# grayhong/self-diagnosing-gan

Hardware: AMD Instinct MI355X
Metric: images/sec (G+D step) (higher is better)
Workload: dtype f32

## Files before the change

self-diagnosing-gan_amd/csrc/train_ops.hip:

```cpp
#include "common.h"

namespace diagan {

enum LossType : int { LOSS_GAN = 0, LOSS_NS = 1, LOSS_HINGE = 2, LOSS_WASSERSTEIN = 3 };

__device__ __forceinline__ float softplus_f(float x) { return fmaxf(x, 0.f) + log1pf(expf(-fabsf(x))); }
__device__ __forceinline__ float sigmoid_f(float x) { return 1.f / (1.f + expf(-x)); }

__device__ __forceinline__ double block_sum_d(double v, double* red) {
  v = wave_sum(v);
  __syncthreads();
  if ((threadIdx.x & 63) == 0) red[threadIdx.x >> 6] = v;
  __syncthreads();
  return (red[0] + red[1]) + (red[2] + red[3]);
}

__global__ __launch_bounds__(256) void d_loss_kernel(const float* __restrict__ real, int n_real,
                                                     const float* __restrict__ fake, int n_fake, int loss_type,
                                                     int gold, float* __restrict__ d_real, float* __restrict__ d_fake,
                                                     float* __restrict__ out) {
  __shared__ double red[4];
  double lr = 0, lf = 0, pr = 0, pf = 0;
  for (int i = threadIdx.x; i < n_real; i += 256) {
    const float x = real[i], s = sigmoid_f(x);
    float l, g;
    if (loss_type == LOSS_HINGE) { l = fmaxf(1.f - x, 0.f); g = x < 1.f ? -1.f : 0.f; }
    else if (loss_type == LOSS_WASSERSTEIN) { l = -x; g = -1.f; }
    else { l = softplus_f(-x); g = s - 1.f; }
    lr += l; pr += s;
    if (d_real) d_real[i] = g / (float)n_real;
  }
  for (int i = threadIdx.x; i < n_fake; i += 256) {
    const float x = fake[i], s = sigmoid_f(x);
    float l, g;
    if (loss_type == LOSS_HINGE) { l = fmaxf(1.f + x, 0.f); g = x > -1.f ? 1.f : 0.f; }
    else if (loss_type == LOSS_WASSERSTEIN) { l = x; g = 1.f; }
    else { l = softplus_f(x); g = s; }
    if (gold) { l *= x; g *= x; }
    lf += l; pf += s;
    if (d_fake) d_fake[i] = g / (float)n_fake;
  }
  lr = block_sum_d(lr, red); lf = block_sum_d(lf, red);
  pr = block_sum_d(pr, red); pf = block_sum_d(pf, red);
  if (threadIdx.x == 0) {
    out[0] = (float)(lr / n_real) + (float)(lf / n_fake);
    out[1] = (float)(pr / n_real);
    out[2] = (float)(pf / n_fake);
  }
}

__global__ __launch_bounds__(256) void g_loss_kernel(const float* __restrict__ fake, int n, int k, int loss_type,
                                                     float* __restrict__ d_fake, float* __restrict__ out) {
  __shared__ double red[4];
  double ls = 0;
  for (int i = threadIdx.x; i < n; i += 256) {
    const float x = fake[i];
    bool sel = true;
    if (k < n) {
      int rank = 0;
      for (int j = 0; j < n; ++j) {
        const float y = fake[j];
        rank += (y > x) || (y == x && j < i);
      }
      sel = rank < k;
    }
    float l = 0.f, g = 0.f;
    if (sel) {
      if (loss_type == LOSS_NS) {
        const float s = sigmoid_f(x);
        l = -logf(s + 1e-8f);
        g = -s * (1.f - s) / (s + 1e-8f);
      } else if (loss_type == LOSS_GAN) {
        l = softplus_f(-x);
        g = sigmoid_f(x) - 1.f;
      }
      else { l = -x; g = -1.f; }
    }
    ls += l;
    if (d_fake) d_fake[i] = g / (float)k;
  }
  ls = block_sum_d(ls, red);
  if (threadIdx.x == 0) out[0] = (float)(ls / k);
}

struct AdamHyper { float lr, beta1, beta2, eps, bc1, bc2_sqrt, grad_scale, pad; };

__global__ __launch_bounds__(256) void adam_kernel(float* __restrict__ p, const float* __restrict__ g,
                                                   float* __restrict__ m, float* __restrict__ v, long n4,
                                                   const AdamHyper h) {
  typedef float f32x4 __attribute__((ext_vector_type(4)));
  const float step_size = h.lr / h.bc1;
  for (long i = (long)blockIdx.x * blockDim.x + threadIdx.x; i < n4; i += (long)gridDim.x * blockDim.x) {
    const f32x4 gv = reinterpret_cast<const f32x4*>(g)[i] * h.grad_scale;
    f32x4 mv = reinterpret_cast<f32x4*>(m)[i], vv = reinterpret_cast<f32x4*>(v)[i], pv = reinterpret_cast<f32x4*>(p)[i];
#pragma unroll
    for (int e = 0; e < 4; ++e) {
      mv[e] = mv[e] + (gv[e] - mv[e]) * (1.f - h.beta1);
      vv[e] = vv[e] * h.beta2 + (1.f - h.beta2) * gv[e] * gv[e];
// ... 78 lines not shown
```

self-diagnosing-gan_amd/diagan/models/base.py:

```python
import os

import torch

from diagan.models.layers import FlatNet
from diagan.ops import eltwise as E


PREFETCH_FAKES = os.environ.get("DIAGAN_PREFETCH_FAKES", "1") != "0"
STACK_G_STEP = os.environ.get("DIAGAN_STACK_G_STEP", "1") != "0"


def _world_size():
    from diagan.trainer import distributed as dist
    return dist.get_world_size()


class BaseModel(FlatNet):

    def restore_checkpoint(self, ckpt_file, optimizer=None):
        if not ckpt_file:
            raise ValueError("No checkpoint file to be restored.")
        ckpt_dict = torch.load(ckpt_file, map_location='cpu', weights_only=False)
        self.load_state_dict(ckpt_dict['model_state_dict'])
        self.param_version += 1
        if optimizer:
            optimizer.load_state_dict(ckpt_dict['optimizer_state_dict'])
        return ckpt_dict['global_step']

    def save_checkpoint(self, directory, global_step, optimizer=None, name=None):
        if not os.path.exists(directory):
            os.makedirs(directory)
        ckpt_dict = {
            'model_state_dict': self.state_dict(),
            'optimizer_state_dict': optimizer.state_dict() if optimizer is not None else None,
            'global_step': global_step,
        }
        if name is None:
            name = "{}_{}_steps.pth".format(os.path.basename(directory), global_step)
        torch.save(ckpt_dict, os.path.join(directory, name))

    def count_params(self):
        return FlatNet.count_params(self)


class BaseGenerator(BaseModel):
    def __init__(self, nz, ngf, bottom_width, loss_type, **kwargs):
        super().__init__()
        self.nz, self.ngf, self.bottom_width, self.loss_type = nz, ngf, bottom_width, loss_type

    def forward(self, x):
        img, _ = self.forward_nhwc(x, self.training, save=False)
        return E.nhwc_to_nchw(img, self.out_channels)

    def generate_images(self, num_images, device=None, noise=None):
        if device is None:
            device = self.device
        if noise is None:
            noise = torch.randn((num_images, self.nz), device=device)
        return self.forward(noise)

    def generate_images_nhwc(self, num_images, device=None, noise=None, save=False, out=None):
        if device is None:
            device = self.device
        if noise is None and not save:
            ready = self._take_prefetched(num_images)
            if ready is not None:
                if out is not None:
                    out.copy_(ready)
                    ready = out
                return ready, None
        if noise is None and save and out is None:
            ready = getattr(self, '_g_step_ready', None)
            self._g_step_ready = None
            if ready is not None and ready[0].shape[0] == num_images and ready[2] == self.param_version and self.training:
                return ready[0], ready[1]
        if noise is None:
            noise = torch.randn((num_images, self.nz), device=device)
        return self.forward_nhwc(noise, self.training, save=save, out=out)

    supports_stacked_forward = False
    max_stacked_images = 0

    def prefetch_fakes(self, count, batch_size, device=None, g_step=False):
        self._fake_pool, self._g_step_ready = [], None
        if not (self.supports_stacked_forward and self.training and count > 1 and PREFETCH_FAKES):
            return
        device = self.device if device is None else device
        per_chunk = min(count, self.max_stacked_images // max(batch_size, 1))
        if per_chunk < 2:
            return
        if g_step and STACK_G_STEP and (count + 1) * batch_size <= self.max_stacked_images:
            noise = [torch.randn((batch_size, self.nz), device=device) for _ in range(count + 1)]
            imgs, ctx = self.forward_nhwc(torch.cat(noise), True, save=True, groups=count + 1, save_group=count)
            parts = imgs.split(batch_size)
            self._fake_pool.extend(parts[:count])
            self._fake_pool_version = self.param_version
            self._g_step_ready = (parts[count], ctx, self.param_version)
            return
        noise = [torch.randn((batch_size, self.nz), device=device) for _ in range(count)]
        for lo in range(0, count, per_chunk):
            part = noise[lo: lo + per_chunk]
            imgs, _ = self.forward_nhwc(torch.cat(part), True, save=False, groups=len(part))
            self._fake_pool.extend(imgs.split(batch_size))
        self._fake_pool_version = self.param_version

    def _take_prefetched(self, num_images):
        pool = getattr(self, '_fake_pool', None)
        if not pool:
            return None
        if pool[0].shape[0] != num_images or self._fake_pool_version != self.param_version or not self.training:
            self._fake_pool = []
            return None
        return pool.pop(0)

    def compute_gan_loss(self, output):
        k = None
        if getattr(self, 'use_topk', False):
            k = int(self.topk_rate * output.shape[0])
        errG, _ = E.loss_gen(output.detach().contiguous(), self.loss_type, k=k, need_grad=False)
        return errG[0]

    def adversarial_grads(self, real_batch, netD, optG, device=None, noise=None):
        self.zero_grad()
        self.wgrad_batch.hold = _world_size() > 1
        batch_size = real_batch[0].shape[0]
        fake, gctx = self.generate_images_nhwc(batch_size, device=device, noise=noise, save=True)
        output, dctx = netD.forward_nhwc(fake, netD.training, save=True, need_dgrad=True, need_in_dgrad=True)
        k = None
        if getattr(self, 'use_topk', False):
            k = int(self.topk_rate * batch_size)
        errG, dlogit = E.loss_gen(output, self.loss_type, k=k)
        g_img = netD.backward_nhwc(dctx, dlogit, need_wgrad=False, need_gx=True)
        self.backward_nhwc(gctx, g_img)
        self.sync_grads(optG)
        return errG

    def train_step(self, real_batch, netD, optG, log_data, device=None, global_step=None, scaler=None, noise=None,
                   **kwargs):
        if scaler is not None:
            raise NotImplementedError("amp/GradScaler is not part of the fp32 MI355X path")
        errG = self.adversarial_grads(real_batch, netD, optG, device=device, noise=noise)
        optG.step()
        log_data.add_metric('errG', errG[0], group='loss')
        return log_data


class BaseDiscriminator(BaseModel):
    supports_defer_step = True

    def __init__(self, ndf, loss_type, **kwargs):
        super().__init__()
        self.ndf, self.loss_type = ndf, loss_type
        self.use_gold = False

    def to_nhwc(self, x):
        return E.nchw_to_nhwc(x.to(dtype=torch.float32), self.in_channels_padded)

    def forward(self, x):
        logit, _ = self.forward_nhwc(self.to_nhwc(x), self.training, save=False, need_dgrad=False)
        return logit

    def compute_gan_loss(self, output_real, output_fake):
        out3, _, _ = E.loss_dis(output_real.detach().contiguous(), output_fake.detach().contiguous(),
                                self.loss_type, gold=self.use_gold, need_grad=False)
        return out3[0]

    def compute_probs(self, output_real, output_fake):
        out3, _, _ = E.loss_dis(output_real.detach().contiguous(), output_fake.detach().contiguous(),
                                self.loss_type, gold=False, need_grad=False)
        return out3[1].item(), out3[2].item()

    def train_step(self, real_batch, netG, optD, log_data, device=None, global_step=None, scaler=None, noise=None,
                   **kwargs):
        if scaler is not None:
            raise NotImplementedError("amp/GradScaler is not part of the fp32 MI355X path")
        self.zero_grad()
        self.wgrad_batch.hold = _world_size() > 1
        real_images = real_batch[0]
        batch_size = real_images.shape[0]
        if getattr(self, 'pair_forward', False) and self.training:
            B, _, H, W = real_images.shape
            x_all = torch.empty((2 * B, H, W, self.in_channels_padded), dtype=torch.float32, device=real_images.device)
            E.nchw_to_nhwc(real_images.to(dtype=torch.float32), self.in_channels_padded, out=x_all[:B])
            netG.generate_images_nhwc(batch_size, device=device, noise=noise, save=False, out=x_all[B:])
            out_all, ctx = self.forward_nhwc(x_all, True, save=True, need_dgrad=True, need_in_dgrad=False, slot='pair')
            dl = torch.empty(2 * B, dtype=torch.float32, device=x_all.device)
            out3, _, _ = E.loss_dis(out_all[:B], out_all[B:], self.loss_type, gold=self.use_gold, d_real=dl[:B],
                                    d_fake=dl[B:])
            self.backward_nhwc(ctx, dl, need_wgrad=True, need_gx=False)
        else:
            out_real, ctx_r = self.forward_nhwc(self.to_nhwc(real_images), self.training, save=True, need_dgrad=True,
                                                need_in_dgrad=False)
            fake, _ = netG.generate_images_nhwc(batch_size, device=device, noise=noise, save=False)
            out_fake, ctx_f = self.forward_nhwc(fake, self.training, save=True, need_dgrad=True, need_in_dgrad=False,
                                                slot=1)
            out3, d_real, d_fake = E.loss_dis(out_real, out_fake, self.loss_type, gold=self.use_gold)
            self.backward_nhwc(ctx_r, d_real, need_wgrad=True, need_gx=False)
            self.backward_nhwc(ctx_f, d_fake, need_wgrad=True, need_gx=False)
        defer = bool(kwargs.get('defer_step', False))
        self.sync_grads(optD, async_op=defer)
        if not defer:
            optD.step()
        log_data.add_metric('errD', out3[0], group='loss')
        log_data.add_metric('D(x)', out3[1], group='prob')
        log_data.add_metric('D(G(z))', out3[2], group='prob')
        return log_data
```

self-diagnosing-gan_amd/diagan/models/layers.py:

```python

import os

import torch
import torch.nn as nn

from diagan.ops import conv as C
from diagan.ops import eltwise as E

WGRAD_BOX = os.environ.get("DIAGAN_WGRAD_BOX", "1") != "0"


def _r4(n):
    return (n + 3) // 4 * 4


class ConvLayer(nn.Module):

    def __init__(self, kind, in_ch, out_ch, ksize, stride=1, pad=0, bias=True, sn=False, xavier_gain=None):
        super().__init__()
        self.kind, self.in_ch, self.out_ch, self.ksize = kind, in_ch, out_ch, ksize
        self.Cip, self.Cop = _r4(in_ch), _r4(out_ch)
        self.geom = C.Geom(kind, self.Cip, self.Cop, ksize, ksize, stride, pad)
        self.sn = sn
        ref = (nn.Conv2d if kind == 'conv' else nn.ConvTranspose2d)(in_ch, out_ch, ksize, stride, pad, bias=bias)
# ... 278 lines not shown
        return self

    def _perm(self, w):
        return w.view(self.ch, self.bw * self.bw, -1).permute(1, 0, 2).reshape(self.ch * self.bw * self.bw, -1)

    def _unperm(self, w):
        return w.view(self.bw * self.bw, self.ch, -1).permute(1, 0, 2).reshape(self.ch * self.bw * self.bw, -1)

    def _pack(self, w):
        out = torch.zeros((w.shape[0], self.geom.Kp), dtype=w.dtype, device=w.device)
        out[:, : self.nz] = self._perm(w)
        return out

    @staticmethod
    def _sd_hook(module, sd, prefix, local_metadata):
        sd[prefix + 'weight'] = module._unperm(sd[prefix + 'weight'][:, : module.nz]).contiguous()
        sd[prefix + 'bias'] = module._unperm(sd[prefix + 'bias'].view(-1, 1)).view(-1).contiguous()
        return sd

    def _load_hook(self, sd, prefix, *args):
        k = prefix + 'weight'
        if k in sd:
            sd[k] = self._pack(sd[k].to(torch.float32))
        if prefix + 'bias' in sd:
            sd[prefix + 'bias'] = self._perm(sd[prefix + 'bias'].to(torch.float32).view(-1, 1)).view(-1).contiguous()
        net = getattr(self, '_net', None)
        if net is not None:
            net.param_version += 1

    def fwd(self, z):
        B = z.shape[0]
        if self.nzp != self.nz:
            z = torch.nn.functional.pad(z, (0, self.nzp - self.nz))
        x = z.contiguous().view(B, 1, 1, self.nzp)
        y = C.conv_fwd(self.geom, x, self.weight.data, bias=self.bias.data)
        return x, y.view(B, self.bw, self.bw, self.ch)

    sn = False

    def wgrad(self, x, dy, slot=0):
        B = x.shape[0]
        dy2 = dy.reshape(B, 1, 1, -1)
        net = getattr(self, '_net', None)
        if net is not None:
            net.wgrad_batch.launch(self, slot, dy2, x, None, None)
            return
        C.conv_wgrad(self.geom, dy2, x, self.weight.grad, accumulate=True)
        E.colsum(dy2, self.bias.grad, accumulate=True)


class HeadLinear(nn.Module):

    def __init__(self, in_ch, sn=True, xavier_gain=None):
        super().__init__()
        self.in_ch, self.sn = in_ch, sn
        ref = nn.Linear(in_ch, 1)
        if xavier_gain is not None:
            nn.init.xavier_uniform_(ref.weight.data, xavier_gain)
        self.weight = nn.Parameter(ref.weight.data.clone())
        self.bias = nn.Parameter(torch.cat([ref.bias.data, torch.zeros(3)]))
        if sn:
            self.register_buffer('sn_u', torch.randn(1, 1))
            self.register_buffer('sn_sigma', torch.ones(1))
        self._register_state_dict_hook(self._sd_hook)
        self._register_load_state_dict_pre_hook(self._load_hook)

    def xavier_(self, gain):
        w = torch.empty(1, self.in_ch)
        nn.init.xavier_uniform_(w, gain)
        self.weight.data.copy_(w.to(self.weight.device))
        return self

    @staticmethod
    def _sd_hook(module, sd, prefix, local_metadata):
        sd[prefix + 'bias'] = sd[prefix + 'bias'][:1].clone()
        return sd

    def _load_hook(self, sd, prefix, *args):
        k = prefix + 'bias'
        if k in sd and sd[k].numel() == 1:
            sd[k] = torch.cat([sd[k].to(torch.float32), torch.zeros(3, device=sd[k].device)])

    class Ctx:
        __slots__ = ("u", "v", "state", "x", "pooled", "_keep", "pair")

        def __init__(self):
            self.pair = None

    def fwd(self, x, training, slot=None):
        ctx = HeadLinear.Ctx()
        inv = None
        if self.sn and slot == 'pair':
            p0, p1 = self._slot_ctx[0], self._slot_ctx[1]
            ctx.pair = (p0, p1)
            ctx.x = x
            ctx.pooled, logit = E.head_fwd(x, self.weight.data, p0.state[1:], self.bias.data, inv_sigma1=p1.state[1:])
            return ctx, logit
        if self.sn and slot is not None:
            pre = self._slot_ctx[slot]
            ctx.u, ctx.v, ctx.state = pre.u, pre.v, pre.state
            inv = ctx.state[1:]
        elif self.sn:
            ctx.u, ctx.v, ctx.state = C.sn_power_iter(self.weight.data, self.sn_u.view(-1), self.sn_sigma,
                                                      training=training)
            inv = ctx.state[1:]
        ctx.x = x
        ctx.pooled, logit = E.head_fwd(x, self.weight.data, inv, self.bias.data)
        return ctx, logit

    def bwd(self, ctx, dlogit, need_wgrad=True):
        if ctx.pair is not None:
            from diagan import _native as nat
            p0, p1 = ctx.pair
            gx, _, _ = E.head_bwd(dlogit, self.weight.data, p0.state[1:], ctx.x, ctx.pooled, need_gx=True,
                                  need_wgrad=False, inv_sigma1=p1.state[1:])
            if need_wgrad:
                h = dlogit.numel() // 2
                for p, sl in ((p0, slice(0, h)), (p1, slice(h, 2 * h))):
                    _, G, dot = E.head_bwd(dlogit[sl], self.weight.data, None, ctx.x[sl], ctx.pooled[sl], need_gx=False,
                                           need_wgrad=True, dbias=self.bias.grad)
                    nat.call("diagan_sn_grad_fix", nat.ptr(G), nat.ptr(dot), 1, nat.ptr(p.u), nat.ptr(p.v),
                             nat.ptr(p.state), nat.ptr(self.weight.grad), 1, self.in_ch, 1, nat.current_stream())
            return gx
        inv = ctx.state[1:] if self.sn else None
        gx, G, dot = E.head_bwd(dlogit, self.weight.data, inv, ctx.x, ctx.pooled, need_gx=True,
                                need_wgrad=need_wgrad, dbias=self.bias.grad if need_wgrad else None)
        if need_wgrad:
            if self.sn:
                from diagan import _native as nat
                nat.call("diagan_sn_grad_fix", nat.ptr(G), nat.ptr(dot), 1, nat.ptr(ctx.u), nat.ptr(ctx.v),
                         nat.ptr(ctx.state), nat.ptr(self.weight.grad), 1, self.in_ch, 1, nat.current_stream())
            else:
                E.add(self.weight.grad.view(-1), G, out=self.weight.grad.view(-1))
        return gx


class SNBatch:

    def __init__(self, net, layers, n_slots=2):
        import numpy as np
        from diagan import _native as nat
        self.net, self.layers, self.nat = net, layers, nat
        dev = net.flat_params.device
        self.slab_generation = net.slab_generation
        desc = np.dtype([('p', np.uint64, 9), ('i', np.int32, 6)])
        self.tables = []
        f32 = dict(dtype=torch.float32, device=dev)
        dims = []
        for slot in range(n_slots):
            tab = np.zeros(len(layers), dtype=desc)
            for li, m in enumerate(layers):
                if isinstance(m, ConvLayer):
                    g = m.geom
                    Co, Ci, RS, Kp, Kd = g.Co, g.Ci, g.R * g.S, g.Kp, g.Kd
                    wf, wd = torch.zeros((Co, Kp), **f32), torch.zeros((Ci, Kd), **f32)
                    ctx = ConvLayer.Ctx()
                else:
                    Co, Ci, RS, Kp, Kd = 1, m.in_ch, 1, m.in_ch, 0
                    wf = wd = None
                    ctx = HeadLinear.Ctx()
                ctx.u, ctx.v, ctx.state = torch.zeros(Co, **f32), torch.zeros(Kp, **f32), torch.ones(2, **f32)
                if isinstance(m, ConvLayer):
                    ctx.wf, ctx.wd, ctx.wkey = wf, wd, slot
                work = torch.zeros(8 * Kp + Co, **f32)
                ctx._keep = (work,)
                if not hasattr(m, '_slot_ctx') or m._slot_ctx is None or len(m._slot_ctx) != n_slots:
                    m._slot_ctx = [None] * n_slots
                m._slot_ctx[slot] = ctx
                ptrs = [m.weight.data.data_ptr(), m.sn_u.data_ptr(), m.sn_sigma.data_ptr(), ctx.u.data_ptr(),
                        ctx.v.data_ptr(), ctx.state.data_ptr(), work.data_ptr(),
                        wf.data_ptr() if wf is not None else 0, wd.data_ptr() if wd is not None else 0]
                tab[li]['p'] = ptrs
                tab[li]['i'] = [Co, Ci, RS, Kp, Kd, 0]
                dims.append((Co, Ci, RS, Kp))
            self.tables.append(torch.from_numpy(tab.view(np.uint8).copy()).to(dev))
        self.max = [max(d[k] for d in dims) for k in range(4)]
        convs = [m for m in layers if isinstance(m, ConvLayer)]
        self.unit = torch.ones(2, **f32)
        ptab = np.zeros(len(convs), dtype=desc)
        for li, m in enumerate(convs):
            g = m.geom
            wd_raw = torch.zeros((g.Ci, g.Kd), **f32)
            pc = ConvLayer.Ctx()
            pc.wf, pc.wd = m.weight.data, wd_raw
            pc.u = pc.v = pc.state = None
            pc.row_scale = (m._slot_ctx[0].state[1:], m._slot_ctx[1].state[1:])
            pc.pair = (m._slot_ctx[0], m._slot_ctx[1])
            pc.wkey = 'pair'
            m._pair_ctx = pc
            ptab[li]['p'] = [m.weight.data.data_ptr(), 0, 0, 0, 0, self.unit.data_ptr(), 0, 0, wd_raw.data_ptr()]
            ptab[li]['i'] = [g.Co, g.Ci, g.R * g.S, g.Kp, g.Kd, 0]
        self.pair_table = torch.from_numpy(ptab.view(np.uint8).copy()).to(dev)
        self.n_convs = len(convs)
# ... 359 lines not shown
```

self-diagnosing-gan_amd/diagan/models/sngan.py:

```python
import math

import torch.nn as nn

from diagan.models.base import BaseDiscriminator, BaseGenerator
from diagan.models.layers import BatchNorm, ConvLayer, HeadLinear, LatentLinear, SNBatch
from diagan.ops import conv as C
from diagan.ops import eltwise as E

RELU = (C.PRO_RELU, None, None)


def _bn_pro(bn):
    return (C.PRO_AFFINE_RELU, bn.scale, bn.shift, bn.group_imgs)


class GBlock(nn.Module):
    def __init__(self, in_channels, out_channels, hidden_channels=None, upsample=False):
        super().__init__()
        hidden_channels = hidden_channels if hidden_channels is not None else out_channels
        self.learnable_sc = in_channels != out_channels or upsample
        self.upsample = upsample
        self.c1 = ConvLayer('conv', in_channels, hidden_channels, 3, 1, 1)
        self.c2 = ConvLayer('conv', hidden_channels, out_channels, 3, 1, 1)
        self.b1 = BatchNorm(in_channels)
# ... 205 lines not shown
            bctx.append(c)
        k = self._last_conv.prepare(training, need_dgrad=save)
        y_pre = self._last_conv.fwd(k, h, pro=_bn_pro(bn))
        y = E.tanh_fwd(y_pre, out=out)
        if save and groups > 1:
            b = z.shape[0] // groups
            sl = slice(save_group * b, (save_group + 1) * b)
            ctx = dict(x0=x0[sl], bctx=bctx, h=h[sl], bn=E.bn_ctx_group(bn, save_group), k=k, y=y[sl])
        else:
            ctx = dict(x0=x0, bctx=bctx, h=h, bn=bn, k=k, y=y) if save else None
        return y, ctx

    def backward_nhwc(self, ctx, g_img):
        g_pre = E.tanh_bwd(ctx['y'], g_img)
        self.wino_batch(('d', None)).prepare(self.param_version)
        h = ctx['h']
        self._last_conv.wgrad(ctx['k'], g_pre, h, pro=_bn_pro(ctx['bn']))
        g_a = self._last_conv.dgrad(ctx['k'], g_pre, h.shape[1:3])
        g = self._last_bn.bwd(g_a, h, ctx['bn'], relu=True)
        for blk, c in zip(reversed(self._blocks()), reversed(ctx['bctx'])):
            g = blk.backward(c, g)
        self.l1.wgrad(ctx['x0'], g)
        self.wgrad_batch.finish(0)


class SNGANGenerator32(SNGANBaseGenerator):
    max_stacked_images = 1536

    def __init__(self, nz=128, ngf=256, bottom_width=4, loss_type='hinge', **kwargs):
        super().__init__(nz=nz, ngf=ngf, bottom_width=bottom_width, loss_type=loss_type, **kwargs)
        self.l1 = LatentLinear(nz, ngf, bottom_width)
        self.block2 = GBlock(ngf, ngf, upsample=True)
        self.block3 = GBlock(ngf, ngf, upsample=True)
        self.block4 = GBlock(ngf, ngf, upsample=True)
        self.b5 = BatchNorm(ngf)
        self.c5 = ConvLayer('conv', ngf, 3, 3, 1, 1)
        self.l1.xavier_(1.0)
        self.c5.xavier_(1.0)
        self._link_layers()

    def _blocks(self):
        return [self.block2, self.block3, self.block4]

    @property
    def _last_bn(self):
        return self.b5

    @property
    def _last_conv(self):
        return self.c5


class SNGANGenerator64(SNGANBaseGenerator):
    max_stacked_images = 768

    def __init__(self, nz=128, ngf=1024, bottom_width=4, loss_type='hinge', **kwargs):
        super().__init__(nz=nz, ngf=ngf, bottom_width=bottom_width, loss_type=loss_type, **kwargs)
        self.l1 = LatentLinear(nz, ngf, bottom_width)
        self.block2 = GBlock(ngf, ngf >> 1, upsample=True)
        self.block3 = GBlock(ngf >> 1, ngf >> 2, upsample=True)
        self.block4 = GBlock(ngf >> 2, ngf >> 3, upsample=True)
        self.block5 = GBlock(ngf >> 3, ngf >> 4, upsample=True)
        self.b6 = BatchNorm(ngf >> 4)
        self.c6 = ConvLayer('conv', ngf >> 4, 3, 3, 1, 1)
        self.l1.xavier_(1.0)
        self.c6.xavier_(1.0)
        self._link_layers()

    def _blocks(self):
        return [self.block2, self.block3, self.block4, self.block5]

    @property
    def _last_bn(self):
        return self.b6

    @property
    def _last_conv(self):
        return self.c6


class SNGANBaseDiscriminator(BaseDiscriminator):
    in_channels_padded = 4
    pair_forward = True

    def _blocks(self):
        raise NotImplementedError

    def _sn_prepare(self, slot, training, need_dgrad):
        sb = getattr(self, '_sn_batch', None)
        if sb is None or sb.stale():
            layers = [m for m in self.modules() if isinstance(m, ConvLayer) and m.sn] + [self._head]
            sb = SNBatch(self, layers)
            object.__setattr__(self, '_sn_batch', sb)
        if slot == 'pair':
            sb.run_pair(training, need_dgrad)
        else:
            sb.run(slot, training, 1 if need_dgrad else 0)

    def forward_nhwc(self, x, training, save=True, need_dgrad=True, need_in_dgrad=True, slot=0):
        self._sn_prepare(slot, training, need_dgrad)
        self.wino_batch(('f', slot)).prepare(self._wino_version(slot))
        blocks = self._blocks()
        h, c0 = blocks[0].forward(x, training, save=save, need_dgrad=need_dgrad, need_in_dgrad=need_in_dgrad,
                                  slot=slot)
        bctx = [c0]
        for blk in blocks[1:]:
            h, c = blk.forward(h, training, save=save, need_dgrad=need_dgrad, slot=slot)
            bctx.append(c)
        hctx, logit = self._head.fwd(h, training, slot=slot)
        return logit, (dict(bctx=bctx, hctx=hctx, slot=slot) if save else None)

    def _wino_version(self, slot):
        sb = self._sn_batch
        return ('p', self.param_version) if slot == 'pair' else sb.slot_ver.get(slot)

    def backward_nhwc(self, ctx, dlogit, need_wgrad=True, need_gx=False):
        self.wino_batch(('d', ctx['slot'])).prepare(self._wino_version(ctx['slot']))
        g = self._head.bwd(ctx['hctx'], dlogit, need_wgrad=need_wgrad)
        blocks = self._blocks()
        for i in range(len(blocks) - 1, -1, -1):
            g = blocks[i].backward(ctx['bctx'][i], g, need_wgrad=need_wgrad, need_gx=(need_gx or i > 0))
        if need_wgrad:
            self.wgrad_batch.finish(ctx['slot'])
        return g


class SNGANDiscriminator32(SNGANBaseDiscriminator):
    def __init__(self, ndf=128, loss_type='hinge', **kwargs):
        super().__init__(ndf=ndf, loss_type=loss_type, **kwargs)
        self.block1 = DBlockOptimized(3, ndf)
        self.block2 = DBlock(ndf, ndf, downsample=True)
        self.block3 = DBlock(ndf, ndf, downsample=False)
        self.block4 = DBlock(ndf, ndf, downsample=False)
        self.l5 = HeadLinear(ndf, sn=True)
        self.l5.xavier_(1.0)
        self._link_layers()

    def _blocks(self):
        return [self.block1, self.block2, self.block3, self.block4]

    @property
    def _head(self):
        return self.l5


class SNGANDiscriminator64(SNGANBaseDiscriminator):
    def __init__(self, ndf=1024, loss_type='hinge', **kwargs):
        super().__init__(ndf=ndf, loss_type=loss_type, **kwargs)
        self.block1 = DBlockOptimized(3, ndf >> 4)
        self.block2 = DBlock(ndf >> 4, ndf >> 3, downsample=True)
        self.block3 = DBlock(ndf >> 3, ndf >> 2, downsample=True)
        self.block4 = DBlock(ndf >> 2, ndf >> 1, downsample=True)
        self.block5 = DBlock(ndf >> 1, ndf, downsample=True)
        self.l6 = HeadLinear(ndf, sn=True)
        self.l6.xavier_(1.0)
        self._link_layers()

    def _blocks(self):
        return [self.block1, self.block2, self.block3, self.block4, self.block5]

    @property
    def _head(self):
        return self.l6
```

self-diagnosing-gan_amd/diagan/ops/eltwise.py:

```python
import torch

from diagan import _native as nat

LOSS_TYPES = {'gan': 0, 'ns': 1, 'hinge': 2, 'wasserstein': 3}
ptr, st = nat.ptr, nat.current_stream


def _f32(shape, dev):
    return torch.empty(shape, dtype=torch.float32, device=dev)


_ws = {}
_ws_retired = []


def _workspace(dev, nbytes):
    w = _ws.get(dev.index)
    if w is None or w.numel() < nbytes:
        if w is not None:
            _ws_retired.append(w)
        w = torch.empty(max(int(nbytes), 1 << 20), dtype=torch.uint8, device=dev)
        _ws[dev.index] = w
    return w


def _colred_ws(dev, M, C, groups=1):
    return _workspace(dev, nat.fn("diagan_colred_workspace")(M, C) * groups)


def nchw_to_nhwc(x, Cp, out=None):
    B, C, H, W = x.shape
    if out is None:
        out = _f32((B, H, W, Cp), x.device)
    nat.call("diagan_nchw_to_nhwc", ptr(x.contiguous()), ptr(out), B, C, H, W, Cp, st())
    return out


def nhwc_to_nchw(x, C):
    B, H, W, Cp = x.shape
    out = _f32((B, C, H, W), x.device)
    nat.call("diagan_nhwc_to_nchw", ptr(x), ptr(out), B, C, H, W, Cp, st())
    return out


def tanh_fwd(x, out=None):
    y = torch.empty_like(x) if out is None else out
    nat.call("diagan_tanh_fwd", ptr(x), ptr(y), x.numel(), st())
    return y


def tanh_bwd(y, g):
    gx = torch.empty_like(y)
    nat.call("diagan_tanh_bwd", ptr(y), ptr(g), ptr(gx), y.numel(), st())
    return gx


class BNCtx:
    __slots__ = ("mean", "invstd", "scale", "shift", "M", "C", "training", "group_imgs")


def _bn_ctx(C, M, training, groups, group_imgs, dev):
    buf = _f32((4, groups, C) if groups > 1 else (4, C), dev)
    ctx = BNCtx()
    ctx.mean, ctx.invstd, ctx.scale, ctx.shift, ctx.M, ctx.C = buf[0], buf[1], buf[2], buf[3], M, C
    ctx.training, ctx.group_imgs = bool(training), (group_imgs if groups > 1 else 0)
    return ctx


def bn_ctx_group(ctx, g):
    if ctx is None or not ctx.group_imgs:
        return ctx
    out = BNCtx()
    out.mean, out.invstd, out.scale, out.shift = ctx.mean[g], ctx.invstd[g], ctx.scale[g], ctx.shift[g]
    out.M, out.C, out.training, out.group_imgs = ctx.M, ctx.C, ctx.training, 0
    return out


def bn_stats(x, gamma, beta, running_mean, running_var, training, eps=1e-5, momentum=0.1, groups=1):
    C = x.shape[-1]
    M = x.numel() // C
    if x.shape[0] % groups:
        raise RuntimeError(f"bn_stats: batch of {x.shape[0]} does not split into {groups} groups")
    Mg, bg = M // groups, x.shape[0] // groups
    ctx = _bn_ctx(C, Mg, training, groups, bg, x.device)
    ws = _colred_ws(x.device, Mg, C, groups) if training else None
    if training and groups > 1:
        nat.call("diagan_bn_stats_grouped", ptr(x), Mg, C, groups, ptr(gamma), ptr(beta), eps, momentum, ptr(running_mean),
# ... 17 lines not shown
    splits = nat.fn("diagan_bn_stats_fused_splits")(tg, C, groups)
    ws = torch.empty(groups * splits * 2 * C, dtype=torch.float64, device=gamma.device) if splits > 1 else None
    nat.call("diagan_bn_stats_fused", ptr(partials), tg, Mg, C, ptr(gamma), ptr(beta), eps, momentum,
             ptr(running_mean), ptr(running_var), ptr(ctx.mean), ptr(ctx.invstd), ptr(ctx.scale), ptr(ctx.shift), groups,
             ptr(ws), 0 if ws is None else ws.numel(), st())
    return ctx


def bn_bwd(g, x, ctx, relu, dgamma, dbeta, accumulate, residual=None, slope=0.0, drop=None, drop_scale=1.0):
    dx = torch.empty_like(x)
    coef = _f32((2 * ctx.C,), x.device)
    ws = _colred_ws(x.device, ctx.M, ctx.C)
    nat.call("diagan_bn_bwd", ptr(g), ptr(x), ctx.M, ctx.C, ptr(ctx.scale), ptr(ctx.shift), ptr(ctx.mean),
             ptr(ctx.invstd), 1 if ctx.training else 0, 1 if relu else 0, slope, ptr(drop), drop_scale, ptr(dgamma), ptr(dbeta), 1 if accumulate else 0,
             ptr(residual),
             ptr(dx), ptr(coef), ptr(ws), st())
    return dx


def colsum(x, out, accumulate):
    C = x.shape[-1]
    M = x.numel() // C
    ws = _colred_ws(x.device, M, C)
    nat.call("diagan_colsum", ptr(x), M, C, ptr(out), 1 if accumulate else 0, ptr(ws), st())
    return out


def upsample2x(x, pro=None):
    B, H, W, C = x.shape
    mode, scale, shift, group_imgs = (tuple(pro) + (0,))[:4] if pro is not None else (0, None, None, 0)
    out = _f32((B, 2 * H, 2 * W, C), x.device)
    nat.call("diagan_upsample2x", ptr(x), ptr(out), B, H, W, C, mode, ptr(scale), ptr(shift), group_imgs, st())
    return out


def upsample2x_bwd(g, residual=None):
    B, H2, W2, C = g.shape
    out = _f32((B, H2 // 2, W2 // 2, C), g.device)
    nat.call("diagan_upsample2x_bwd", ptr(g), ptr(out), B, H2 // 2, W2 // 2, C, ptr(residual), st())
    return out


def boxsum2(x, relu_in=False):
    B, H, W, C = x.shape
    out = _f32((B, H + 1, W + 1, C), x.device)
    nat.call("diagan_boxsum2", ptr(x), ptr(out), B, H, W, C, 1 if relu_in else 0, st())
    return out


def avgpool2(x, residual=None, relu_in=False):
    B, H, W, C = x.shape
    out = _f32((B, H // 2, W // 2, C), x.device)
    nat.call("diagan_avgpool2", ptr(x), ptr(out), B, H, W, C, ptr(residual), 1 if relu_in else 0, st())
    return out


def avgpool2_bwd(g, residual=None):
    B, Ho, Wo, C = g.shape
    out = _f32((B, 2 * Ho, 2 * Wo, C), g.device)
    nat.call("diagan_avgpool2_bwd", ptr(g), ptr(out), B, 2 * Ho, 2 * Wo, C, ptr(residual), st())
    return out


def head_fwd(x, w, inv_sigma, bias, inv_sigma1=None):
    B, H, W, C = x.shape
    pooled = _f32((B, C), x.device)
    logit = _f32((B, 1), x.device)
    nat.call("diagan_head_fwd", ptr(x), ptr(w), ptr(inv_sigma), ptr(inv_sigma1), B // 2, ptr(bias), ptr(pooled),
             ptr(logit), B, H * W, C, st())
    return pooled, logit


def head_bwd(dlogit, w, inv_sigma, x, pooled, need_gx=True, need_wgrad=True, dbias=None, accumulate_bias=True,
             inv_sigma1=None):
    B, H, W, C = x.shape
    gx = torch.empty_like(x) if need_gx else None
    G = _f32((C,), x.device) if need_wgrad else None
    dot = torch.empty(1, dtype=torch.float64, device=x.device) if need_wgrad else None
    nat.call("diagan_head_bwd", ptr(dlogit), ptr(w), ptr(inv_sigma), ptr(inv_sigma1), B // 2, ptr(x), ptr(pooled),
             ptr(gx), ptr(G), ptr(dot), ptr(dbias), 1 if accumulate_bias else 0, B, H * W, C, st())
    return gx, G, dot


def act_fwd(x, slope, scale=None, shift=None, drop=None, drop_scale=1.0):
    C = x.shape[-1]
    out = torch.empty_like(x)
    nat.call("diagan_act_fwd", ptr(x), ptr(scale), ptr(shift), slope, ptr(drop), drop_scale, ptr(out), x.numel() // C, C, st())
    return out


def act_bwd(g, x, slope, drop=None, drop_scale=1.0):
    out = torch.empty_like(x)
    nat.call("diagan_act_bwd", ptr(g), ptr(x), slope, ptr(drop), drop_scale, ptr(out), x.numel(), st())
    return out


def linear1_fwd(x, w, bias):
    B, C = x.shape
    logit = _f32((B, 1), x.device)
    nat.call("diagan_linear1_fwd", ptr(x), ptr(w), ptr(bias), ptr(logit), B, C, st())
    return logit


def linear1_wgrad(dlogit, x, dw, dbias):
    B, C = x.shape
    nat.call("diagan_linear1_wgrad", ptr(dlogit), ptr(x), ptr(dw), ptr(dbias), B, C, st())


def linear1_bwd_input(dlogit, w, B, C):
    gx = _f32((B, C), w.device)
    nat.call("diagan_linear1_bwd_input", ptr(dlogit), ptr(w), ptr(gx), B, C, st())
    return gx


def add(a, b, out=None):
    out = torch.empty_like(a) if out is None else out
    nat.call("diagan_add", ptr(a), ptr(b), ptr(out), a.numel(), st())
    return out


def loss_dis(out_real, out_fake, loss_type, gold=False, need_grad=True, d_real=None, d_fake=None):
    dev = out_real.device
    nr, nf = out_real.numel(), out_fake.numel()
    if need_grad and d_real is None:
        d_real, d_fake = _f32((nr,), dev), _f32((nf,), dev)
    out3 = _f32((3,), dev)
    nat.call("diagan_loss_dis", ptr(out_real), nr, ptr(out_fake), nf, LOSS_TYPES[loss_type], 1 if gold else 0,
             ptr(d_real), ptr(d_fake), ptr(out3), st())
    return out3, d_real, d_fake


def loss_gen(out_fake, loss_type, k=None, need_grad=True):
    dev = out_fake.device
    n = out_fake.numel()
    k = n if k is None else k
    d_fake = _f32((n,), dev) if need_grad else None
    out1 = _f32((1,), dev)
    nat.call("diagan_loss_gen", ptr(out_fake), n, k, LOSS_TYPES[loss_type], ptr(d_fake), ptr(out1), st())
    return out1, d_fake


def adam_step(p, g, m, v, lr, beta1, beta2, eps, step, grad_scale=1.0):
    bc1 = 1.0 - beta1 ** step
    bc2_sqrt = (1.0 - beta2 ** step) ** 0.5
    nat.call("diagan_adam_step", ptr(p), ptr(g), ptr(m), ptr(v), p.numel(), lr, beta1, beta2, eps, bc1, bc2_sqrt,
             grad_scale, st())


def adam_hyper_row(lr, beta1, beta2, eps, step, grad_scale=1.0):
    return [lr, beta1, beta2, eps, 1.0 - beta1 ** step, (1.0 - beta2 ** step) ** 0.5, grad_scale, 0.0]


def adam_step_dev(p, g, m, v, hyper_row):
    nat.call("diagan_adam_step_dev", ptr(p), ptr(g), ptr(m), ptr(v), p.numel(), ptr(hyper_row), st())
```

Baseline: 5354.

## Fuse discriminator head forward, loss, and input-gradient into one kernel

Adds a head_fused kernel that, per image, does ReLU-sum pooling, the linear logit with spectral-norm scaling, the loss gradient, and the head's input gradient in a single launch. A head_finish kernel then reduces the loss scalars and computes the weight/bias gradient with the spectral-norm correction. This replaces the separate head forward, loss, and head backward launches for both the D and G steps. It is meant to cut kernel launches and re-reads of the head activation, at the cost of a single-block finish kernel and a new ABI path.

```diff
diff --git a/include/diagan_head.h b/include/diagan_head.h
--- /dev/null
+++ b/include/diagan_head.h
@@ -0,0 +1,22 @@
+#ifndef DIAGAN_HEAD_H
+#define DIAGAN_HEAD_H
+
+#include <stdint.h>
+
+#ifdef __cplusplus
+extern "C" {
+#endif
+
+int diagan_head_fused(const float* x, const float* w, const float* inv_sigma, const float* inv_sigma1, int split_b, const float* bias,
+                      int kind, int loss_type, int gold, int n_real, float* pooled, float* logit, float* dlogit, float* gx, int B, int HW,
+                      int C, void* stream);
+
+int diagan_head_finish(const float* logit, const float* dlogit, const float* pooled, const float* w, int B, int C, int kind,
+                       int loss_type, int gold, int n_real, float* out, int halves, int split_b, const float* u0, const float* v0,
+                       const float* state0, const float* u1, const float* v1, const float* state1, float* wgrad, float* bgrad,
+                       void* stream);
+
+#ifdef __cplusplus
+}
+#endif
+#endif
diff --git a/self-diagnosing-gan_amd/csrc/head_fused.hip b/self-diagnosing-gan_amd/csrc/head_fused.hip
--- /dev/null
+++ b/self-diagnosing-gan_amd/csrc/head_fused.hip
@@ -0,0 +1,267 @@
+#include "loss_math.h"
+
+namespace diagan {
+
+typedef float f32x4 __attribute__((ext_vector_type(4)));
+constexpr int HF_T = 256;
+enum HeadKind : int { HEAD_D = 0, HEAD_G = 1 };
+
+__device__ __forceinline__ void dis_real_terms(float x, int loss_type, float& l, float& g, float& s) {
+  s = sigmoid_f(x);
+  if (loss_type == LOSS_HINGE) { l = fmaxf(1.f - x, 0.f); g = x < 1.f ? -1.f : 0.f; }
+  else if (loss_type == LOSS_WASSERSTEIN) { l = -x; g = -1.f; }
+  else { l = softplus_f(-x); g = s - 1.f; }
+}
+__device__ __forceinline__ void dis_fake_terms(float x, int loss_type, int gold, float& l, float& g, float& s) {
+  s = sigmoid_f(x);
+  if (loss_type == LOSS_HINGE) { l = fmaxf(1.f + x, 0.f); g = x > -1.f ? 1.f : 0.f; }
+  else if (loss_type == LOSS_WASSERSTEIN) { l = x; g = 1.f; }
+  else { l = softplus_f(x); g = s; }
+  if (gold) { l *= x; g *= x; }
+}
+__device__ __forceinline__ void gen_terms(float x, int loss_type, float& l, float& g) {
+  if (loss_type == LOSS_NS) {
+    const float s = sigmoid_f(x);
+    l = -logf(s + 1e-8f);
+    g = -s * (1.f - s) / (s + 1e-8f);
+  } else if (loss_type == LOSS_GAN) {
+    l = softplus_f(-x);
+    g = sigmoid_f(x) - 1.f;
+  }
+  else { l = -x; g = -1.f; }
+}
+
+__global__ __launch_bounds__(HF_T) void head_fused_kernel(const float* __restrict__ x, const float* __restrict__ w,
+                                                          const float* __restrict__ inv_sigma,
+                                                          const float* __restrict__ inv_sigma1, int split_b,
+                                                          const float* __restrict__ bias, int kind, int loss_type, int gold,
+                                                          int n_real, float* pooled, float* __restrict__ logit,
+                                                          float* __restrict__ dlogit, float* __restrict__ gx, int HW, int C) {
+  __shared__ float red[HF_T][4];
+  __shared__ float sd;
+  const int b = blockIdx.x, B = gridDim.x;
+  const int C4 = C >> 2;
+  const int CW = C4 < 64 ? C4 : 64, RL = HF_T / CW;
+  const int cc = threadIdx.x % CW, rl = threadIdx.x / CW;
+  const f32x4* xb = reinterpret_cast<const f32x4*>(x) + (long)b * HW * C4;
+  for (int c0 = 0; c0 < C4; c0 += CW) {
+    const int c4 = c0 + cc;
+    f32x4 s = {0.f, 0.f, 0.f, 0.f};
+    if (c4 < C4 && rl < RL)
+      for (int r = rl; r < HW; r += RL) {
+        const f32x4 v = xb[(long)r * C4 + c4];
+#pragma unroll
+        for (int e = 0; e < 4; ++e) s[e] += fmaxf(v[e], 0.f);
+      }
+#pragma unroll
+    for (int e = 0; e < 4; ++e) red[threadIdx.x][e] = s[e];
+    __syncthreads();
+    if (rl == 0 && c4 < C4) {
+      f32x4 t = {0.f, 0.f, 0.f, 0.f};
+      for (int k = 0; k < RL; ++k)
+#pragma unroll
+        for (int e = 0; e < 4; ++e) t[e] += red[k * CW + cc][e];
+      reinterpret_cast<f32x4*>(pooled)[(long)b * C4 + c4] = t;
+    }
+    __syncthreads();
+  }
+  if (threadIdx.x < 64) {
+    const int lane = threadIdx.x;
+    float s = 0.f;
+    for (int c = lane; c < C; c += 64) s = fmaf(pooled[(long)b * C + c], w[c], s);
+    s = wave_sum(s);
+    if (lane == 0) {
+      const float* ip = (inv_sigma1 && b >= split_b) ? inv_sigma1 : inv_sigma;
+      const float inv = ip ? ip[0] : 1.f;
+      const float z = s * inv + (bias ? bias[0] : 0.f);
+      float l, g, sg;
+      if (kind == HEAD_G) {
+        gen_terms(z, loss_type, l, g);
+        g = g / (float)B;
+      } else if (b < n_real) {
+        dis_real_terms(z, loss_type, l, g, sg);
+        g = g / (float)n_real;
+      } else {
+        dis_fake_terms(z, loss_type, gold, l, g, sg);
+        g = g / (float)(B - n_real);
+      }
+      logit[b] = z;
+      dlogit[b] = g;
+      sd = g * inv;
+    }
+  }
+  __syncthreads();
+  const float d = sd;
+  f32x4* gb = reinterpret_cast<f32x4*>(gx) + (long)b * HW * C4;
+  const int n4 = HW * C4;
+#pragma unroll 4
+  for (int i = threadIdx.x; i < n4; i += HF_T) {
+    const f32x4 xv = xb[i];
+    const f32x4 wv = reinterpret_cast<const f32x4*>(w)[i % C4];
+    f32x4 o;
+#pragma unroll
+    for (int e = 0; e < 4; ++e) o[e] = xv[e] > 0.f ? d * wv[e] : 0.f;
+    gb[i] = o;
+  }
+}
+
+struct HeadFinishArgs {
+  const float *logit, *dlogit, *pooled, *w;
+  const float *u0, *v0, *state0, *u1, *v1, *state1;
+  float *out, *wgrad, *bgrad;
+  int B, C, kind, loss_type, gold, n_real, halves, split_b;
+};
+
+__global__ __launch_bounds__(3 * HF_T) void head_finish_kernel(const HeadFinishArgs a) {
+  extern __shared__ float Gs[];
+  __shared__ double red[3][4][4];
+  __shared__ float sb[2];
+  const int grp = threadIdx.x >> 8, t = threadIdx.x & (HF_T - 1), wave = t >> 6;
+  const int B = a.B, C = a.C;
+  double acc[4] = {0.0, 0.0, 0.0, 0.0};
+  int nsum = 1;
+  const float *v = nullptr, *state = nullptr;
+  float* Gh = nullptr;
+  float inv = 1.f, u = 0.f;
+  if (grp == 0) {
+    if (a.kind == HEAD_G) {
+      for (int i = t; i < B; i += HF_T) {
+        float l, g;
+        gen_terms(a.logit[i], a.loss_type, l, g);
+        acc[0] += l;
+      }
+    } else {
+      nsum = 4;
+      const int n_real = a.n_real, n_fake = B - a.n_real;
+      const float* fake = a.logit + n_real;
+      for (int i = t; i < n_real; i += HF_T) {
+        float l, g, s;
+        dis_real_terms(a.logit[i], a.loss_type, l, g, s);
+        acc[0] += l; acc[2] += s;
+      }
+      for (int i = t; i < n_fake; i += HF_T) {
+        float l, g, s;
+        dis_fake_terms(fake[i], a.loss_type, a.gold, l, g, s);
+        acc[1] += l; acc[3] += s;
+      }
+    }
+  } else {
+    const int h = grp - 1;
+    const int lo = h ? a.split_b : 0, hi = (h + 1 < a.halves) ? a.split_b : B, nb = hi - lo;
+    const float* dl = a.dlogit + lo;
+    const float* pl = a.pooled + (long)lo * C;
+    state = h ? a.state1 : a.state0;
+    v = h ? a.v1 : a.v0;
+    Gh = Gs + (long)h * C;
+    if (state) { inv = state[1]; u = (h ? a.u1 : a.u0)[0]; }
+    if (t == HF_T - 1) {
+      float s = 0.f;
+      for (int b = 0; b < nb; ++b) s += dl[b];
+      sb[h] = s;
+    }
+    for (int c = t; c < C; c += HF_T) {
+      float s = 0.f;
+#pragma unroll 32
+      for (int b = 0; b < nb; ++b) s = fmaf(dl[b], pl[(long)b * C + c], s);
+      Gh[c] = s;
+      acc[0] += (double)s * a.w[c];
+    }
+  }
+#pragma unroll
+  for (int k = 0; k < 4; ++k)
+    if (k < nsum) {
+      const double r = wave_sum(acc[k]);
+      if ((t & 63) == 0) red[grp][k][wave] = r;
+    }
+  __syncthreads();
+  if (grp == 0) {
+    if (t == 0) {
+      double sum[4];
+#pragma unroll
+      for (int k = 0; k < 4; ++k) sum[k] = (red[0][k][0] + red[0][k][1]) + (red[0][k][2] + red[0][k][3]);
+      if (a.kind == HEAD_G) a.out[0] = (float)(sum[0] / B);
+      else {
+        const int n_real = a.n_real, n_fake = B - a.n_real;
+        a.out[0] = (float)(sum[0] / n_real) + (float)(sum[1] / n_fake);
+        a.out[1] = (float)(sum[2] / n_real);
+        a.out[2] = (float)(sum[3] / n_fake);
+      }
+    }
+  } else if (state) {
+    const double dot = (red[grp][0][0] + red[grp][0][1]) + (red[grp][0][2] + red[grp][0][3]);
+    double sdot = 0.0;
+    sdot += dot;
+    const float coef = (float)(sdot * (double)inv);
+    const float un = u * coef;
+    for (int c = t; c < C; c += HF_T) {
+#pragma clang fp contract(off)
+      Gh[c] = __builtin_fmaf(-un, v[c], Gh[c]) * inv;
+    }
+  }
+  __syncthreads();
+  if (!a.wgrad) return;
+  for (int c = threadIdx.x; c < C; c += blockDim.x) {
+    float o = Gs[c] + a.wgrad[c];
+    if (a.halves == 2) o = Gs[C + c] + o;
+    a.wgrad[c] = o;
+  }
+  if (threadIdx.x == 0) {
+    float o = a.bgrad[0] + sb[0];
+    if (a.halves == 2) o = o + sb[1];
+    a.bgrad[0] = o;
+  }
+}
+
+}
+
+using namespace diagan;
+
+#define ST ((hipStream_t)stream)
+
+static int head_loss_args_ok(const char* what, int kind, int loss_type, int gold, int n_real, int B) {
+  DG_REQUIRE(kind == HEAD_D || kind == HEAD_G, "%s: unknown kind %d (0 discriminator, 1 generator)", what, kind);
+  DG_REQUIRE(loss_type >= 0 && loss_type <= 3, "%s: unknown loss type %d", what, loss_type);
+  DG_REQUIRE(kind == HEAD_G || (n_real > 0 && n_real < B), "%s: the discriminator loss needs 0 < n_real < B (n_real=%d B=%d)",
+             what, n_real, B);
+  DG_REQUIRE(!gold || (kind == HEAD_D && (loss_type == LOSS_NS || loss_type == LOSS_HINGE || loss_type == LOSS_GAN)),
+             "%s: GOLD re-weighting exists for the discriminator's 'ns' and 'hinge' losses only", what);
+  return DIAGAN_OK;
+}
+
+DIAGAN_API int diagan_head_fused(const float* x, const float* w, const float* inv_sigma, const float* inv_sigma1, int split_b,
+                                 const float* bias, int kind, int loss_type, int gold, int n_real, float* pooled,
+                                 float* logit, float* dlogit, float* gx, int B, int HW, int C, void* stream) {
+  DG_REQUIRE(x && w && pooled && logit && dlogit && gx && B > 0 && HW > 0 && C > 0 && (C & 3) == 0, "head_fused: bad args");
+  DG_REQUIRE((long)HW * C / 4 < (1L << 31), "head_fused: one image must hold fewer than 2^31 float4");
+  DG_REQUIRE(!inv_sigma1 || (inv_sigma && split_b > 0 && split_b < B), "head_fused: a second 1/sigma needs the first and 0 < split_b < B");
+  if (int rc = head_loss_args_ok("head_fused", kind, loss_type, gold, n_real, B)) return rc;
+  hipLaunchKernelGGL(head_fused_kernel, dim3(B), dim3(HF_T), 0, ST, x, w, inv_sigma, inv_sigma1, inv_sigma1 ? split_b : B,
+                     bias, kind, loss_type, gold, n_real, pooled, logit, dlogit, gx, HW, C);
+  return check_launch("head_fused");
+}
+
+DIAGAN_API int diagan_head_finish(const float* logit, const float* dlogit, const float* pooled, const float* w, int B, int C,
+                                  int kind, int loss_type, int gold, int n_real, float* out, int halves, int split_b,
+                                  const float* u0, const float* v0, const float* state0, const float* u1, const float* v1,
+                                  const float* state1, float* wgrad, float* bgrad, void* stream) {
+  DG_REQUIRE(logit && out && B > 0 && C > 0, "head_finish: bad args");
+  if (int rc = head_loss_args_ok("head_finish", kind, loss_type, gold, n_real, B)) return rc;
+  if (wgrad) {
+    DG_REQUIRE(dlogit && pooled && w && bgrad, "head_finish: the weight gradient needs dlogit, pooled, w and bgrad");
+    DG_REQUIRE(C <= 8192, "head_finish: the weight gradient keeps C floats per half in LDS, C <= 8192 (C=%d)", C);
+    DG_REQUIRE(halves == 1 || (halves == 2 && split_b > 0 && split_b < B), "head_finish: halves is 1, or 2 with 0 < split_b < B");
+    DG_REQUIRE(!u0 == !v0 && !u0 == !state0, "head_finish: u, v and state of a half are given together");
+    DG_REQUIRE(halves == 1 ? (!u1 && !v1 && !state1) : (!u1 == !u0 && !v1 == !u0 && !state1 == !u0),
+               "head_finish: both halves with spectral norm or neither; no second half's u, v, state without a second half");
+  }
+  HeadFinishArgs a;
+  a.logit = logit; a.dlogit = dlogit; a.pooled = pooled; a.w = w;
+  a.u0 = u0; a.v0 = v0; a.state0 = state0;
+  a.u1 = u1; a.v1 = v1; a.state1 = state1;
+  a.out = out; a.wgrad = wgrad; a.bgrad = bgrad;
+  a.B = B; a.C = C; a.kind = kind; a.loss_type = loss_type; a.gold = gold; a.n_real = n_real;
+  a.halves = halves; a.split_b = split_b;
+  const int groups = wgrad ? 1 + halves : 1;
+  hipLaunchKernelGGL(head_finish_kernel, dim3(1), dim3(groups * HF_T), wgrad ? (size_t)halves * C * sizeof(float) : 0, ST, a);
+  return check_launch("head_finish");
+}
diff --git a/self-diagnosing-gan_amd/csrc/loss_math.h b/self-diagnosing-gan_amd/csrc/loss_math.h
--- /dev/null
+++ b/self-diagnosing-gan_amd/csrc/loss_math.h
@@ -0,0 +1,19 @@
+#pragma once
+#include "common.h"
+
+namespace diagan {
+
+enum LossType : int { LOSS_GAN = 0, LOSS_NS = 1, LOSS_HINGE = 2, LOSS_WASSERSTEIN = 3 };
+
+__device__ __forceinline__ float softplus_f(float x) { return fmaxf(x, 0.f) + log1pf(expf(-fabsf(x))); }
+__device__ __forceinline__ float sigmoid_f(float x) { return 1.f / (1.f + expf(-x)); }
+
+__device__ __forceinline__ double block_sum_d(double v, double* red) {
+  v = wave_sum(v);
+  __syncthreads();
+  if ((threadIdx.x & 63) == 0) red[threadIdx.x >> 6] = v;
+  __syncthreads();
+  return (red[0] + red[1]) + (red[2] + red[3]);
+}
+
+}
diff --git a/self-diagnosing-gan_amd/csrc/train_ops.hip b/self-diagnosing-gan_amd/csrc/train_ops.hip
--- a/self-diagnosing-gan_amd/csrc/train_ops.hip
+++ b/self-diagnosing-gan_amd/csrc/train_ops.hip
@@ -1,19 +1,6 @@
-#include "common.h"
+#include "loss_math.h"
 
 namespace diagan {
-
-enum LossType : int { LOSS_GAN = 0, LOSS_NS = 1, LOSS_HINGE = 2, LOSS_WASSERSTEIN = 3 };
-
-__device__ __forceinline__ float softplus_f(float x) { return fmaxf(x, 0.f) + log1pf(expf(-fabsf(x))); }
-__device__ __forceinline__ float sigmoid_f(float x) { return 1.f / (1.f + expf(-x)); }
-
-__device__ __forceinline__ double block_sum_d(double v, double* red) {
-  v = wave_sum(v);
-  __syncthreads();
-  if ((threadIdx.x & 63) == 0) red[threadIdx.x >> 6] = v;
-  __syncthreads();
-  return (red[0] + red[1]) + (red[2] + red[3]);
-}
 
 __global__ __launch_bounds__(256) void d_loss_kernel(const float* __restrict__ real, int n_real,
                                                      const float* __restrict__ fake, int n_fake, int loss_type,
diff --git a/self-diagnosing-gan_amd/diagan/_native/head_abi.py b/self-diagnosing-gan_amd/diagan/_native/head_abi.py
--- /dev/null
+++ b/self-diagnosing-gan_amd/diagan/_native/head_abi.py
@@ -0,0 +1,35 @@
+import os
+
+from diagan import _native as nat
+from diagan._native import parse_header
+
+HEADER_PATH = os.path.join(os.path.dirname(nat.HEADER_PATH), "diagan_head.h")
+
+_sigs = None
+_bound = {}
+
+
+def signatures():
+    global _sigs
+    if _sigs is None:
+        if not os.path.exists(HEADER_PATH):
+            raise RuntimeError(f"diagan_head.h not found at {HEADER_PATH}: the ctypes signatures are read from it "
+                               "(the package runs from a checkout of the repository).")
+        with open(HEADER_PATH) as f:
+            _sigs = parse_header(f.read())
+    return _sigs
+
+
+def fn(name):
+    f = _bound.get(name)
+    if f is None:
+        f = getattr(nat.lib(), name)
+        f.restype, f.argtypes = signatures()[name]
+        _bound[name] = f
+    return f
+
+
+def call(name, *args):
+    rc = fn(name)(*args)
+    if rc != 0:
+        raise RuntimeError(f"{name} failed ({rc}): {nat.last_error()}")
diff --git a/self-diagnosing-gan_amd/diagan/models/base.py b/self-diagnosing-gan_amd/diagan/models/base.py
--- a/self-diagnosing-gan_amd/diagan/models/base.py
+++ b/self-diagnosing-gan_amd/diagan/models/base.py
@@ -8,6 +8,7 @@
 
 PREFETCH_FAKES = os.environ.get("DIAGAN_PREFETCH_FAKES", "1") != "0"
 STACK_G_STEP = os.environ.get("DIAGAN_STACK_G_STEP", "1") != "0"
+HEAD_FUSED = os.environ.get("DIAGAN_HEAD_FUSED", "1") != "0"
 
 
 def _world_size():
@@ -125,12 +126,19 @@
         self.wgrad_batch.hold = _world_size() > 1
         batch_size = real_batch[0].shape[0]
         fake, gctx = self.generate_images_nhwc(batch_size, device=device, noise=noise, save=True)
-        output, dctx = netD.forward_nhwc(fake, netD.training, save=True, need_dgrad=True, need_in_dgrad=True)
         k = None
         if getattr(self, 'use_topk', False):
             k = int(self.topk_rate * batch_size)
-        errG, dlogit = E.loss_gen(output, self.loss_type, k=k)
-        g_img = netD.backward_nhwc(dctx, dlogit, need_wgrad=False, need_gx=True)
+        fused = HEAD_FUSED and getattr(netD, 'supports_head_loss', False) and (k is None or k == batch_size)
+        if fused:
+            output, dctx = netD.forward_nhwc(fake, netD.training, save=True, need_dgrad=True, need_in_dgrad=True,
+                                             head_loss=('g', self.loss_type, False))
+            g_img = netD.backward_nhwc(dctx, None, need_wgrad=False, need_gx=True)
+            errG = netD.head_loss_out(dctx)
+        else:
+            output, dctx = netD.forward_nhwc(fake, netD.training, save=True, need_dgrad=True, need_in_dgrad=True)
+            errG, dlogit = E.loss_gen(output, self.loss_type, k=k)
+            g_img = netD.backward_nhwc(dctx, dlogit, need_wgrad=False, need_gx=True)
         self.backward_nhwc(gctx, g_img)
         self.sync_grads(optG)
         return errG
@@ -183,11 +191,17 @@
             x_all = torch.empty((2 * B, H, W, self.in_channels_padded), dtype=torch.float32, device=real_images.device)
             E.nchw_to_nhwc(real_images.to(dtype=torch.float32), self.in_channels_padded, out=x_all[:B])
             netG.generate_images_nhwc(batch_size, device=device, noise=noise, save=False, out=x_all[B:])
-            out_all, ctx = self.forward_nhwc(x_all, True, save=True, need_dgrad=True, need_in_dgrad=False, slot='pair')
-            dl = torch.empty(2 * B, dtype=torch.float32, device=x_all.device)
-            out3, _, _ = E.loss_dis(out_all[:B], out_all[B:], self.loss_type, gold=self.use_gold, d_real=dl[:B],
-                                    d_fake=dl[B:])
-            self.backward_nhwc(ctx, dl, need_wgrad=True, need_gx=False)
+            if HEAD_FUSED and getattr(self, 'supports_head_loss', False):
+                out_all, ctx = self.forward_nhwc(x_all, True, save=True, need_dgrad=True, need_in_dgrad=False, slot='pair',
+                                                 head_loss=('d', self.loss_type, self.use_gold))
+                self.backward_nhwc(ctx, None, need_wgrad=True, need_gx=False)
+                out3 = self.head_loss_out(ctx)
+            else:
+                out_all, ctx = self.forward_nhwc(x_all, True, save=True, need_dgrad=True, need_in_dgrad=False, slot='pair')
+                dl = torch.empty(2 * B, dtype=torch.float32, device=x_all.device)
+                out3, _, _ = E.loss_dis(out_all[:B], out_all[B:], self.loss_type, gold=self.use_gold, d_real=dl[:B],
+                                        d_fake=dl[B:])
+                self.backward_nhwc(ctx, dl, need_wgrad=True, need_gx=False)
         else:
             out_real, ctx_r = self.forward_nhwc(self.to_nhwc(real_images), self.training, save=True, need_dgrad=True,
                                                 need_in_dgrad=False)
diff --git a/self-diagnosing-gan_amd/diagan/models/layers.py b/self-diagnosing-gan_amd/diagan/models/layers.py
--- a/self-diagnosing-gan_amd/diagan/models/layers.py
+++ b/self-diagnosing-gan_amd/diagan/models/layers.py
@@ -384,18 +384,21 @@
             sd[k] = torch.cat([sd[k].to(torch.float32), torch.zeros(3, device=sd[k].device)])
 
     class Ctx:
-        __slots__ = ("u", "v", "state", "x", "pooled", "_keep", "pair")
+        __slots__ = ("u", "v", "state", "x", "pooled", "_keep", "pair", "head_loss", "logit", "dlogit", "gx", "loss_out")
 
         def __init__(self):
             self.pair = None
-
-    def fwd(self, x, training, slot=None):
+            self.head_loss = None
+
+    def fwd(self, x, training, slot=None, head_loss=None):
         ctx = HeadLinear.Ctx()
         inv = None
         if self.sn and slot == 'pair':
             p0, p1 = self._slot_ctx[0], self._slot_ctx[1]
             ctx.pair = (p0, p1)
             ctx.x = x
+            if head_loss is not None:
+                return ctx, self._fwd_fused(ctx, x, head_loss, p0.state[1:], p1.state[1:])
             ctx.pooled, logit = E.head_fwd(x, self.weight.data, p0.state[1:], self.bias.data, inv_sigma1=p1.state[1:])
             return ctx, logit
         if self.sn and slot is not None:
@@ -407,10 +410,32 @@
                                                       training=training)
             inv = ctx.state[1:]
         ctx.x = x
+        if head_loss is not None:
+            return ctx, self._fwd_fused(ctx, x, head_loss, inv, None)
         ctx.pooled, logit = E.head_fwd(x, self.weight.data, inv, self.bias.data)
         return ctx, logit
 
+    def _fwd_fused(self, ctx, x, head_loss, inv, inv1):
+        kind, loss_type, gold = head_loss
+        ctx.head_loss = head_loss
+        ctx.pooled, ctx.logit, ctx.dlogit, ctx.gx = E.head_fused(x, self.weight.data, inv, self.bias.data, kind, loss_type, gold=gold,
+                                                                 n_real=x.shape[0] // 2 if kind == 'd' else 0, inv_sigma1=inv1)
+        return ctx.logit
+
+    def _bwd_fused(self, ctx, need_wgrad):
+        kind, loss_type, gold = ctx.head_loss
+        if ctx.pair is not None:
+            halves = [(p.u, p.v, p.state) for p in ctx.pair]
+        else:
+            halves = [(ctx.u, ctx.v, ctx.state) if self.sn else None]
+        ctx.loss_out = E.head_finish(ctx.logit, ctx.dlogit, ctx.pooled, self.weight.data, kind, loss_type, gold=gold,
+                                     n_real=ctx.logit.shape[0] // 2 if kind == 'd' else 0, halves=halves,
+                                     wgrad=self.weight.grad if need_wgrad else None, bgrad=self.bias.grad if need_wgrad else None)
+        return ctx.gx
+
     def bwd(self, ctx, dlogit, need_wgrad=True):
+        if ctx.head_loss is not None:
+            return self._bwd_fused(ctx, need_wgrad)
         if ctx.pair is not None:
             from diagan import _native as nat
             p0, p1 = ctx.pair
diff --git a/self-diagnosing-gan_amd/diagan/models/sngan.py b/self-diagnosing-gan_amd/diagan/models/sngan.py
--- a/self-diagnosing-gan_amd/diagan/models/sngan.py
+++ b/self-diagnosing-gan_amd/diagan/models/sngan.py
@@ -311,6 +311,7 @@
 class SNGANBaseDiscriminator(BaseDiscriminator):
     in_channels_padded = 4
     pair_forward = True
+    supports_head_loss = True
 
     def _blocks(self):
         raise NotImplementedError
@@ -326,7 +327,7 @@
         else:
             sb.run(slot, training, 1 if need_dgrad else 0)
 
-    def forward_nhwc(self, x, training, save=True, need_dgrad=True, need_in_dgrad=True, slot=0):
+    def forward_nhwc(self, x, training, save=True, need_dgrad=True, need_in_dgrad=True, slot=0, head_loss=None):
         self._sn_prepare(slot, training, need_dgrad)
         self.wino_batch(('f', slot)).prepare(self._wino_version(slot))
         blocks = self._blocks()
@@ -336,8 +337,12 @@
         for blk in blocks[1:]:
             h, c = blk.forward(h, training, save=save, need_dgrad=need_dgrad, slot=slot)
             bctx.append(c)
-        hctx, logit = self._head.fwd(h, training, slot=slot)
+        hctx, logit = self._head.fwd(h, training, slot=slot, head_loss=head_loss if save else None)
         return logit, (dict(bctx=bctx, hctx=hctx, slot=slot) if save else None)
+
+    @staticmethod
+    def head_loss_out(ctx):
+        return ctx['hctx'].loss_out
 
     def _wino_version(self, slot):
         sb = self._sn_batch
diff --git a/self-diagnosing-gan_amd/diagan/ops/eltwise.py b/self-diagnosing-gan_amd/diagan/ops/eltwise.py
--- a/self-diagnosing-gan_amd/diagan/ops/eltwise.py
+++ b/self-diagnosing-gan_amd/diagan/ops/eltwise.py
@@ -1,8 +1,10 @@
 import torch
 
 from diagan import _native as nat
+from diagan._native import head_abi as hnat
 
 LOSS_TYPES = {'gan': 0, 'ns': 1, 'hinge': 2, 'wasserstein': 3}
+HEAD_KINDS = {'d': 0, 'g': 1}
 ptr, st = nat.ptr, nat.current_stream
 
 
@@ -186,6 +188,26 @@
     return gx, G, dot
 
 
+def head_fused(x, w, inv_sigma, bias, kind, loss_type, gold=False, n_real=0, inv_sigma1=None):
+    B, H, W, C = x.shape
+    pooled, logit, dlogit, gx = _f32((B, C), x.device), _f32((B, 1), x.device), _f32((B,), x.device), torch.empty_like(x)
+    hnat.call("diagan_head_fused", ptr(x), ptr(w), ptr(inv_sigma), ptr(inv_sigma1), B // 2, ptr(bias), HEAD_KINDS[kind],
+              LOSS_TYPES[loss_type], 1 if gold else 0, n_real, ptr(pooled), ptr(logit), ptr(dlogit), ptr(gx), B, H * W, C, st())
+    return pooled, logit, dlogit, gx
+
+
+def head_finish(logit, dlogit, pooled, w, kind, loss_type, gold=False, n_real=0, halves=None, wgrad=None, bgrad=None):
+    B, C = pooled.shape
+    out = _f32((3 if kind == 'd' else 1,), logit.device)
+    sn, nh = (None,) * 6, 1
+    if wgrad is not None:
+        nh = len(halves)
+        sn = tuple(ptr(t) for h in (tuple(halves) + (None,))[:2] for t in (h if h is not None else (None,) * 3))
+    hnat.call("diagan_head_finish", ptr(logit), ptr(dlogit), ptr(pooled), ptr(w), B, C, HEAD_KINDS[kind], LOSS_TYPES[loss_type],
+              1 if gold else 0, n_real, ptr(out), nh, B // 2, *sn, ptr(wgrad), ptr(bgrad), st())
+    return out
+
+
 def act_fwd(x, slope, scale=None, shift=None, drop=None, drop_scale=1.0):
     C = x.shape[-1]
     out = torch.empty_like(x)
```

After: 5398 (median of 6 runs). No clear change (+0.8%).
